# rensonnetg/microstructure_fingerprinting

Hardware: AMD Instinct MI355X
Metric: voxels/sec, 2-fascicle exhaustive NNLS, 782-atom x 200-measurement dictionary (higher is better)
Workload: dtype f64 (pairs ranked on split-f16 MFMA, short list re-evaluated in f64); 1 GPU; C2: 100000 voxels/GPU, 2 fascicles, 782 atoms x 200 measurements; voxels_per_gpu=100000, global_voxels=100000, atoms=782, measurements=200, ranks_in_group=1

## Files before the change

microstructure_fingerprinting_amd/csrc/fit_k2s.hip:

```cpp
#pragma once
#include "fit_k2.hip"

typedef _Float16 h8 __attribute__((ext_vector_type(8)));
typedef _Float16 h4 __attribute__((ext_vector_type(4)));
typedef float f32x16 __attribute__((ext_vector_type(16)));
typedef float f32x2 __attribute__((ext_vector_type(2)));
typedef float f32x4 __attribute__((ext_vector_type(4)));
typedef int i32x4 __attribute__((ext_vector_type(4)));

#ifndef MFX_S_DC
#define MFX_S_DC 1.5e-5
#endif
template <int KS>
__host__ __device__ constexpr double mfx_s_dc() { return KS <= 13 ? (double)MFX_S_DC : 1.05 * (2.38e-6 + 3.0 * KS * 3.046e-7); }
#define MFX_S_DENMIN 1e-3
#define MFX_S_BOUND 0x40000000
#define MFX_S_GUARD 0.25

__device__ __forceinline__ unsigned long long mfx_nonneg_bits(double x) {
  return (unsigned long long)__double_as_longlong(x > 0.0 ? x : 0.0);
}

template <int CTRL>
__device__ __forceinline__ float mfx_dpp_max_f32(float v) {
// ... 12 lines not shown
  return (double)fmaxf(fmaxf(r0, r1), fmaxf(r2, r3));
}
__device__ __forceinline__ double mfx_rcp_nr(double x) {
  const double r0 = (double)__builtin_amdgcn_rcpf((float)x);
  return fma(r0, fma(-x, r0, 1.0), r0);
}

__device__ __forceinline__ double mfx_readlane_f64(double v, int l) {
  const long long b = __double_as_longlong(v);
  const unsigned lo = (unsigned)__builtin_amdgcn_readlane((int)(b & 0xffffffffll), l);
  const unsigned hi = (unsigned)__builtin_amdgcn_readlane((int)(b >> 32), l);
  return __longlong_as_double((long long)(((unsigned long long)hi << 32) | lo));
}

__device__ __forceinline__ void mfx_split16(float f, _Float16& hi, _Float16& lo) {
  asm("" : "+v"(f));
  const float h = __uint_as_float(__float_as_uint(f) & 0xffffe000u);
  hi = (_Float16)h;
  lo = (_Float16)(f - h);
}

#include "k2s_shared.h"

template <int KS, bool BR = false, int NB = 3, bool XC = false>
__global__ __launch_bounds__(512, 2) void mfx_fit_k2s_kernel(FitK2Args a) {
  constexpr int WG = 512, NW = 8;
  constexpr int MP = KS * 16;
  extern __shared__ double smem[];
  int tid = threadIdx.x;
  const int lane = tid & 63, wave = tid >> 6;
  const int lr = lane & 31, lh = lane >> 5;
  [[maybe_unused]] const int M = a.P.M;
  const int N = a.T.N, ldn = a.T.ldn;
  const int NP = (N + 31) & ~31;
  const int ntiles = NP >> 5;
  const int vox = a.vox_list ? a.vox_list[a.vox_base + blockIdx.x] : a.vox_base + (int)blockIdx.x;

  const K2sLds<KS, NB, BR, XC, NW * 64> L(smem, NP);
  K2S_UNPACK(L);
  const K2sVoxel VX = k2s_prologue<KS, NB, BR, XC, NW * 64, WG>(a, L, vox, tid);
  const double y_sq = VX.y_sq, yx = VX.yx, ramp = VX.ramp, dc_eff = VX.dc_eff, mrg = VX.mrg, etol = VX.etol;
  (void)y_sq; (void)yx;
  const float2* __restrict__ tab32 = a.P.tab32s;
  auto tab32_at = [&](int ro, int n) -> float2 { return *(const float2*)((const char*)tab32 + ((unsigned)(ro + n) << 3)); };
  auto tab32x2_at = [&](int ro, int n) -> f32x4 { return *(const f32x4*)((const char*)tab32 + ((unsigned)(ro + n) << 3)); };
  auto push = [&](double S, int i, int j) { k2s_push(L, a.scap, S, i, j); };

  MFX_STAMP(2);
#ifdef MFX_STAMPS_RND
  if (a.stamps && tid == 0) a.stamps[(size_t)blockIdx.x * 16] = __builtin_amdgcn_s_memtime();
#endif
  double bs1 = 0.0;
  int bn1 = 0;
  const int nrounds = (ntiles + NW - 1) / NW;
#ifdef MFX_EXP_NOAUDIT
  const int aud_key = -1;
#else
  const int aud_key = a.audit ? k2s_audit_key(k2s_audit_hash(vox), (ntiles % NW == 1 && ntiles > 1) ? ntiles - 1 : ntiles, ntiles) : -1;
#endif
  for (int round = 0; round < nrounds; ++round) {
    const bool tail = (ntiles - round * NW == 1) && (ntiles > 1);
    const int rt = tail ? round * NW : round * NW + wave;
    const bool rt_valid = rt < ntiles;
    const int rtc = rt_valid ? rt : 0;
    h8 afh[KS], afl[KS];
    {
      const int n = rtc * 32 + lr;
      const int nn = min(n, ldn - 1);
      double a2 = 0.0, ay = 0.0;
      float um1 = 0.0f;
      if constexpr (XC) um1 = (rt_valid && n < N) ? -s_uf[n] : 0.0f;
      mfx_static_for<0, KS>([&](auto kc) {
        constexpr int ks = decltype(kc)::value;
        float2 d[8];
#pragma unroll
        for (int j = 0; j < 8; ++j) d[j] = tab32_at(s_rs[16 * ks + 8 * lh + j], nn);
        h8 vh, vl;
#pragma unroll
        for (int j = 0; j < 8; ++j) {
          float fv = fmaf(d[j].y, s_t0f[16 * ks + 8 * lh + j], d[j].x);
          fv = rt_valid ? fv : 0.0f;
          if constexpr (XC) {
            if constexpr (ks == KS - 1) { if (j == 7) fv = lh ? um1 : fv; }
          } else {
            const double fd = (double)fv;
            a2 = fma(fd, fd, a2);
            ay = fma((double)s_yf[16 * ks + 8 * lh + j], fd, ay);
          }
          _Float16 x, y;
// ... 36 lines not shown
#ifdef MFX_STAMPS_RND
    int dbg_flagged = 0, dbg_groups = 0;
#endif
    const float DCF = XC ? (float)((mfx_s_dc<KS>() + 2e-6) * ramp) * (1.0f + 2e-7f)
                         : (float)mfx_s_dc<KS>() + 2e-6f;
    auto pq_of = [&](float z, float rth, float& P, float& Q) {
      P = fminf(1.0f, fmaxf(z, 0.0f) * rth);
      Q = __builtin_amdgcn_sqrtf(fmaxf(0.0f, fmaf(-P, P, 1.0f) - 1.2e-7f)) * (1.0f - 3e-7f);
    };
    unsigned long long sc_thr = 0ull;
    float sc_z2 = 0.0f, sc_s = 0.0f;
    auto scan_pre = [&](int ct) {
      const int j = ct * 32 + lr;
      sc_thr = s_thr[0];
      sc_z2 = s_Zf[NP + j];
      sc_s = s_cs[NP + j];
    };
#ifdef MFX_STAMPS_SCAN
    int dbg_calls = 0;
#define MFX_SCAN_T(k) do { if (a.stamps && round == 0 && dbg_calls == 1 && wave == 0 && lane == 0) a.stamps[(size_t)blockIdx.x * 16 + (k)] = __builtin_amdgcn_s_memtime(); } while (0)
#else
#define MFX_SCAN_T(k) do { } while (0)
#endif
    auto scan_main = [&](const f32x16& acc, int ct) {
#ifdef MFX_STAMPS_SCAN
      ++dbg_calls;
#endif
      MFX_SCAN_T(0);
      {
        if (((rt << 8) | ct) == aud_key) {
          const unsigned h = k2s_audit_hash(vox);
          const int ga = (h >> 16) & 15;
          float v = acc[0];
#pragma unroll
          for (int g = 1; g < 16; ++g) v = (ga == g) ? acc[g] : v;
          if (lane == (int)((h >> 20) & 63)) ((float*)(s_red + 30))[0] = v;
        }
      }
      const int j = ct * 32 + lr;
      thr = fmax(thr, __longlong_as_double((long long)sc_thr));
      const float rth = __builtin_amdgcn_rsqf(fmaxf((float)thr * (1.0f - 2e-7f), 1e-30f)) * (1.0f + 4e-7f);
      float* pqw = s_pq + wave * 64;
      if (thr > thr_rows) {
        thr_rows = thr;
        if (lane < 32) {
          const float z1 = s_Zf[rtc * 32 + lane], n1 = s_cs[rtc * 32 + lane];
          float P, Q;
          pq_of(z1, rth, P, Q);
          const bool ok = n1 > 0.0f;
          pqw[lane] = ok ? (P + DCF) * n1 : 0.0f;
          pqw[32 + lane] = ok ? Q * ((1.0f - DCF) * n1) : 1e18f;
        }
      }
      const float z2f = sc_z2, n2 = sc_s;
      float P2, Q2;
      pq_of(z2f, rth, P2, Q2);
      const bool colok = n2 > 0.0f;
      const float p2 = colok ? (P2 + DCF) * n2 : -1e18f, q2 = colok ? Q2 * ((1.0f - DCF) * n2) : 1e18f;
      float mm[4];
#pragma unroll
      for (int q = 0; q < 4; ++q) {
        const f32x4 p1q = *(const f32x4*)(pqw + 8 * q + 4 * lh);
        const f32x4 q1q = *(const f32x4*)(pqw + 32 + 8 * q + 4 * lh);
        float t[4];
#pragma unroll
        for (int u = 0; u < 4; ++u) t[u] = fmaf(-q1q[u], q2, fmaf(p1q[u], p2, -acc[4 * q + u]));
        mm[q] = fmaxf(fmaxf(t[0], t[1]), fmaxf(t[2], t[3]));
      }
      MFX_SCAN_T(1);
      if (__any(fmaxf(fmaxf(mm[0], mm[1]), fmaxf(mm[2], mm[3])) >= 0.0f)) {
        MFX_SCAN_T(2);
#ifdef MFX_STAMPS_RND
        ++dbg_flagged;
#endif
        const double z2 = (double)s_Zf[NP + j], n2d = (double)s_cs[NP + j];
#pragma unroll 1
        for (int q = 0; q < 4; ++q) {
          if (!__any(mm[q] >= 0.0f)) continue;
          const f32x4 p1q = *(const f32x4*)(pqw + 8 * q + 4 * lh);
          const f32x4 q1q = *(const f32x4*)(pqw + 32 + 8 * q + 4 * lh);
#pragma unroll 1
          for (int gg = 0; gg < 4; ++gg) {
            const int g = 4 * q + gg;
            if (!__any(fmaf(-q1q[gg], q2, fmaf(p1q[gg], p2, -acc[g])) >= 0.0f)) continue;
#ifdef MFX_STAMPS_RND
            ++dbg_groups;
#endif
            const int i = rt * 32 + (g & 3) + 8 * (g >> 2) + 4 * lh;
            const double n12 = (double)s_cs[i] * n2d;
            const double c = n12 > 0.0 ? (double)acc[g] * mfx_rcp_nr(n12) : 0.0;
            const double z1 = (double)s_Zf[i];
            const double e1 = fma(-c, z2, z1);
            const double e2 = fma(-c, z1, z2);
            const double den = fma(-c, c, 1.0);
            const double num = fma(z2, e2, z1 * e1);
            const bool pos = (e1 > -etol) & (e2 > -etol);
            const bool wellc = (den >= MFX_S_DENMIN) & (c >= 0.0);
            const bool hit = pos & wellc & (fma(-thr, den, num) >= 0.0);
            const bool near = pos & !wellc;
            if (!__any(hit | near)) continue;
            double S = -1.0;
            if (hit) {
              S = num * mfx_rcp_nr(den);
            } else if (near) {
              const double dlo = den - 2.0 * dc_eff - dc_eff * dc_eff;
              const double u1 = fabs(e1) + etol, u2 = fabs(e2) + etol;
              S = (dlo > 0.0 && c > -0.5) ? fmin(fma(z2, z2, u1 * u1 / dlo), fma(z1, z1, u2 * u2 / dlo)) + mrg : 1e300;
            }
            bool feas = hit;
            double q1x = 0.0, q2x = 0.0;
            if constexpr (XC) {
// ... 24 lines not shown
            const double smax = mfx_wave_max_down(fmax(sraise, 0.0));
            if (smax - 2.0 * mrg > thr) {
              thr = smax - 2.0 * mrg;
              if (lane == 0) atomicMax(&s_thr[0], mfx_nonneg_bits(thr));
            }
            if ((hit | near) && slist >= thr) push(slist, i, hit ? j : (j | MFX_S_BOUND));
#ifdef MFX_STAMPS_SCAN
            if (a.stamps && round == 0 && dbg_calls == 1 && wave == 0 && lane == 0) {
              unsigned long long* st = a.stamps + (size_t)blockIdx.x * 16;
              if (st[15] < 8) st[4 + st[15]] = __builtin_amdgcn_s_memtime();
              ++st[15];
            }
#endif
          }
        }
        MFX_SCAN_T(3);
      }
    };
    auto scan_tile = [&](const f32x16& acc, int ct) { scan_pre(ct); scan_main(acc, ct); };

#ifdef MFX_EXP_NOTAIL
    if (tail) continue;
#endif
    if (tail) {
#ifdef MFX_STAMPS_RND
      if (a.stamps && tid == 0 && round < 4) a.stamps[(size_t)blockIdx.x * 16 + 2 * round + 1] = __builtin_amdgcn_s_memtime();
#endif
      thr = __longlong_as_double((long long)s_thr[0]);
      for (int ct = wave; ct < ntiles; ct += NW) {
        const int n = ct * 32 + lr;
        const int nn = min(n, ldn - 1);
        float tail_u2 = 0.0f;
        if constexpr (XC) tail_u2 = s_uf[NP + n];
        f32x16 acc;
#pragma unroll
        for (int g = 0; g < 16; ++g) acc[g] = 0.0f;
        float2 d[2][8];
#pragma unroll
        for (int j = 0; j < 8; ++j) d[0][j] = tab32_at(s_rs[MP + 8 * lh + j], nn);
        mfx_static_for<0, KS>([&](auto kc) {
          constexpr int ks = decltype(kc)::value;
          if constexpr (ks + 1 < KS) {
#pragma unroll
            for (int j = 0; j < 8; ++j) d[(ks + 1) & 1][j] = tab32_at(s_rs[MP + 16 * (ks + 1) + 8 * lh + j], nn);
          }
          h8 bh, bl;
#pragma unroll
          for (int j = 0; j < 8; ++j) {
            _Float16 x, y;
            float fv = fmaf(d[ks & 1][j].y, s_t0f[MP + 16 * ks + 8 * lh + j], d[ks & 1][j].x);
            if constexpr (XC && ks == KS - 1) { if (j == 7) fv = lh ? tail_u2 : fv; }
            mfx_split16(fv, x, y);
            bh[j] = x; bl[j] = y;
          }
          acc = __builtin_amdgcn_mfma_f32_32x32x16_f16(afh[ks], bh, acc, 0, 0, 0);
          acc = __builtin_amdgcn_mfma_f32_32x32x16_f16(afh[ks], bl, acc, 0, 0, 0);
          acc = __builtin_amdgcn_mfma_f32_32x32x16_f16(afl[ks], bh, acc, 0, 0, 0);
          __builtin_amdgcn_sched_barrier(0);
        });
        scan_tile(acc, ct);
      }
      __syncthreads();
#ifdef MFX_STAMPS_RND
      if (a.stamps && tid == 0 && round < 4) a.stamps[(size_t)blockIdx.x * 16 + 2 * round + 2] = __builtin_amdgcn_s_memtime();
#endif
      continue;
    }

    const int grp = wave >> 2, tg = tid & 255;
    static_assert(KS <= 16, "one generation item per thread");
    f32x4 gd[8];
    const int gq = KS * grp + (tg >> 4);
    const bool gact = (tg >> 4) < KS;
    auto gen_load = [&](int ch) {
      const int nn = min(ch * 32 + 2 * (tg & 15), ldn - 2);
      const int q = gact ? gq : KS * grp;
#pragma unroll
      for (int e = 0; e < 8; ++e) gd[e] = tab32x2_at(s_rs[MP + 8 * q + e], nn);
    };
#ifndef MFX_XC_GT
#define MFX_XC_GT 0
#endif
    constexpr bool GT = KS <= 13 && (!XC || MFX_XC_GT);
    float g_t[GT ? 8 : 1];
    if constexpr (GT) {
#pragma unroll
      for (int e = 0; e < 8; ++e) g_t[e] = s_t0f[MP + 8 * (gact ? gq : KS * grp) + e];
    }
    auto gen_store = [&](int ch, int buf) {
      if (gact) {
        const int c0 = 2 * (tg & 15);
        h8 hi0, lo0, hi1, lo1;
// ... 21 lines not shown
#pragma unroll
    for (int g = 0; g < 16; ++g) acc[g] = 0.0f;
    auto mfma_chunk = [&](int buf) {
#pragma unroll
      for (int g = 0; g < 16; ++g) acc[g] = 0.0f;
      const _Float16* bhp = sBh + buf * KS * 512 + lane * 8;
      const _Float16* blp = sBl + buf * KS * 512 + lane * 8;
      h8 bh = *(const h8*)bhp, bl = *(const h8*)blp;
      mfx_static_for<0, KS>([&](auto kc) {
        constexpr int ks = decltype(kc)::value;
        h8 bhn = bh, bln = bl;
        if constexpr (ks + 1 < KS) {
          bhn = *(const h8*)(bhp + (ks + 1) * 512);
          bln = *(const h8*)(blp + (ks + 1) * 512);
        }
        acc = __builtin_amdgcn_mfma_f32_32x32x16_f16(afh[ks], bh, acc, 0, 0, 0);
        acc = __builtin_amdgcn_mfma_f32_32x32x16_f16(afh[ks], bl, acc, 0, 0, 0);
        acc = __builtin_amdgcn_mfma_f32_32x32x16_f16(afl[ks], bh, acc, 0, 0, 0);
        bh = bhn; bl = bln;
        __builtin_amdgcn_sched_barrier(0);
      });
    };

    if (round == 0) MFX_STAMP(3);
#ifdef MFX_STAMPS_RND
    if (a.stamps && tid == 0 && round < 4) a.stamps[(size_t)blockIdx.x * 16 + 2 * round + 1] = __builtin_amdgcn_s_memtime();
#endif
    if constexpr (NB == 3) {
      gen_load(0);
      gen_store(0, 0);
      if (grp == 0) {
        if (ntiles > 1) { gen_load(1); gen_store(1, 1); }
        if (ntiles > 2) gen_load(2);
      } else if (ntiles > 1) {
        gen_load(1);
      }
      __syncthreads();
      if (round == 0) MFX_STAMP(4);
      thr = __longlong_as_double((long long)s_thr[0]);
      int b0 = 0;
#ifdef MFX_EXP_NOGEN
      const bool exp_gen = round == 0;
#else
      constexpr bool exp_gen = true;
#endif
      for (int c = 0; c <= ntiles; ++c) {
#ifdef MFX_STAMPS_HS
#ifndef MFX_HS_ROUND
#define MFX_HS_ROUND 1
#define MFX_HS_C0 10
#endif
        if (a.stamps && round == MFX_HS_ROUND && c >= MFX_HS_C0 && c < MFX_HS_C0 + 16 && tid == 0) a.stamps[(size_t)blockIdx.x * 16 + c - MFX_HS_C0] = __builtin_amdgcn_s_memtime();
#endif
        const int b1 = b0 == 2 ? 0 : b0 + 1, b2 = b1 == 2 ? 0 : b1 + 1;
        if (grp == 0) {
          if (c < ntiles) {
            if (rt_valid) { mfma_chunk(b0); scan_pre(c); }
            if (exp_gen && c + 2 < ntiles) gen_store(c + 2, b2);
            if (rt_valid) scan_main(acc, c);
            if (exp_gen && c + 3 < ntiles) gen_load(c + 3);
          }
        } else {
          if (c >= 1 && rt_valid) scan_pre(c - 1);
          if (exp_gen && c + 1 < ntiles) gen_store(c + 1, b1);
          if (c >= 1 && rt_valid) scan_main(acc, c - 1);
          if (exp_gen && c + 2 < ntiles) gen_load(c + 2);
          if (c < ntiles && rt_valid) mfma_chunk(b0);
        }
        asm volatile("s_waitcnt lgkmcnt(0)\n\ts_barrier" ::: "memory");
        b0 = b1;
      }
    } else {
      gen_load(0);
      gen_store(0, 0);
      if (grp == 1 && ntiles > 1) { gen_load(1); gen_store(1, 1); }
      __syncthreads();
      if (round == 0) MFX_STAMP(4);
      thr = __longlong_as_double((long long)s_thr[0]);
      for (int hs = 0; hs <= 2 * ntiles; ++hs) {
        if ((hs & 1) == grp) {
          const int c = (hs - grp) >> 1;
          if (c < ntiles) {
            if (c + 1 + grp < ntiles) gen_load(c + 1 + grp);
            if (rt_valid) mfma_chunk(c & 1);
          }
        } else {
          const int c = (hs - 1 - grp) >> 1;
          if (c >= 0 && c < ntiles) {
            if (c + 1 + grp < ntiles) gen_store(c + 1 + grp, (c + 1 + grp) & 1);
            if (rt_valid) scan_tile(acc, c);
          }
        }
        __syncthreads();
      }
    }
    if (round == 0) MFX_STAMP(5);
#ifdef MFX_STAMPS_RND
    if (a.stamps && tid == 0 && round < 4) a.stamps[(size_t)blockIdx.x * 16 + 2 * round + 2] = __builtin_amdgcn_s_memtime();
    if (a.stamps && lane == 0 && round < 3) atomicAdd(&a.stamps[(size_t)blockIdx.x * 16 + 9 + round], (unsigned long long)dbg_flagged + ((unsigned long long)dbg_groups << 32));
#endif
  }
  k2s_finish<KS, NB, BR, XC, NW * 64, WG>(a, L, VX, vox, wave, lane, bs1, bn1);
}
```

microstructure_fingerprinting_amd/csrc/k2s_launch.h:

```cpp
#pragma once
#include "mfx_host.h"
#include "fit_k2s.hip"

template <int KS, bool BR, int NB>
static int launch_k2s_t(const FitK2Args& a, int nvox, hipStream_t st) {
  MfxThread& T = mfx_thread();
  const size_t lds = mfx_k2s_lds_bytes(KS, a.T.N, BR, NB);
  auto kern = mfx_fit_k2s_kernel<KS, BR, NB>;
  HIPCHK(hipFuncSetAttribute((const void*)kern, hipFuncAttributeMaxDynamicSharedMemorySize, (int)lds));
  StreamMem fbm(st);
  HIPCHK(fbm.alloc(sizeof(int) * ((size_t)nvox + 8)));
  int* fb = fbm.as<int>();
  HIPCHK(hipMemsetAsync(fb, 0, 8 * sizeof(int), st));
  if (int rc = mfx_prof_begin(st)) return rc;
  FitK2Args aa = a;
  aa.stamps = T.stamps;
  aa.fb_count = fb;
  aa.fb_list = fb + 8;
  aa.audit = fb + 2;
  aa.scap = T.k2s_cap ? T.k2s_cap : MFX_S_CAP;
  hipLaunchKernelGGL(kern, dim3(nvox), dim3(512), lds, st, aa);
  HIPCHK(hipGetLastError());
  if (int rc = mfx_prof_end(st)) return rc;
  FitK2Args ab = a;
  ab.vox_list = fb + 8;
  ab.list_count = fb;
  if (int rc = mfx_launch_k2_f64(ab, nvox, st, false)) return rc;
  if (int rc = mfx_fb_accumulate(fb, 2, st)) return rc;
  return mfx_fb_accumulate_audit(fb + 2, st);
}

#define MFX_K2S_TU(KS_, NAME_)                                                            \
  int NAME_(const FitK2Args& a, int nvox, hipStream_t st, bool br, int NB) {              \
    if (NB == 3) return br ? launch_k2s_t<KS_, true, 3>(a, nvox, st) : launch_k2s_t<KS_, false, 3>(a, nvox, st); \
    return br ? launch_k2s_t<KS_, true, 2>(a, nvox, st) : launch_k2s_t<KS_, false, 2>(a, nvox, st);              \
  }
```

microstructure_fingerprinting_amd/csrc/k2s_shared.h:

```cpp
#pragma once

template <int KS, int NB, bool BR, bool XC, int PQF>
struct K2sLds {
  static constexpr int MP = KS * 16;
  double* smem;
  _Float16* sBh;
  _Float16* sBl;
  double* s_y;
  double* s_t0;
  double* s_red;
  Cand* s_cand;
  unsigned long long* s_thr;
  int* s_r0;
  int* s_cnt;
  float* s_t0f;
  float* s_Zf;
  float* s_cs;
  float* s_yf;
  float* s_pq;
  double* s_t1;
  double* s_tG;
  double* s_dG;
  int* s_r1;
  int* s_rs;
  int* s_evl4;
  float* s_xf;
  float* s_uf;
  __device__ __forceinline__ K2sLds(double* smem_, int NP) : smem(smem_) {
    sBh = (_Float16*)smem;
    sBl = sBh + NB * KS * 512;
    s_y = (double*)(sBl + NB * KS * 512);
    s_t0 = s_y + MP;
    s_red = s_t0 + 2 * MP;
    s_cand = (Cand*)(s_red + 32);
    s_thr = (unsigned long long*)(s_cand + MFX_S_CAP);
    s_r0 = (int*)(s_thr + 2);
    s_cnt = s_r0 + 2 * MP;
    s_t0f = (float*)(s_cnt + 4);
    s_Zf = s_t0f + 2 * MP;
    s_cs = s_Zf + 2 * NP;
    s_yf = s_cs + 2 * NP;
    s_pq = s_yf + MP;
    s_t1 = (double*)(s_pq + PQF);
    s_tG = s_t1 + (BR ? 2 * MP : 0);
    s_dG = s_tG + (BR ? MP : 0);
    s_r1 = (int*)(s_dG + (BR ? MP : 0));
    s_rs = BR ? s_r1 + 2 * MP : s_r0;
    s_evl4 = s_r1 + (BR ? 4 * MP : 0);
    s_xf = (float*)(s_evl4 + (KS < 8 ? MFX_S_CAP : 0));
    s_uf = s_xf + (XC ? MP : 0);
  }
};
#define K2S_UNPACK(L) \
  [[maybe_unused]] _Float16* const sBh = (L).sBh; \
  [[maybe_unused]] _Float16* const sBl = (L).sBl; \
  [[maybe_unused]] double* const s_y = (L).s_y; \
  [[maybe_unused]] double* const s_t0 = (L).s_t0; \
  [[maybe_unused]] double* const s_red = (L).s_red; \
  [[maybe_unused]] Cand* const s_cand = (L).s_cand; \
  [[maybe_unused]] unsigned long long* const s_thr = (L).s_thr; \
  [[maybe_unused]] int* const s_r0 = (L).s_r0; \
  [[maybe_unused]] int* const s_cnt = (L).s_cnt; \
  [[maybe_unused]] float* const s_t0f = (L).s_t0f; \
  [[maybe_unused]] float* const s_Zf = (L).s_Zf; \
  [[maybe_unused]] float* const s_cs = (L).s_cs; \
  [[maybe_unused]] float* const s_yf = (L).s_yf; \
  [[maybe_unused]] float* const s_pq = (L).s_pq; \
  [[maybe_unused]] double* const s_t1 = (L).s_t1; \
  [[maybe_unused]] double* const s_tG = (L).s_tG; \
  [[maybe_unused]] double* const s_dG = (L).s_dG; \
  [[maybe_unused]] int* const s_r1 = (L).s_r1; \
  [[maybe_unused]] int* const s_rs = (L).s_rs; \
  [[maybe_unused]] int* const s_evl4 = (L).s_evl4; \
// ... 11 lines not shown

__device__ __forceinline__ unsigned k2s_audit_hash(int vox) {
  unsigned h = (unsigned)vox * 2654435761u;
  h ^= h >> 15; h *= 2246822519u; h ^= h >> 13; h *= 3266489917u; h ^= h >> 16;
  return h;
}
__device__ __forceinline__ int k2s_audit_key(unsigned h, int ntiles_reg, int ntiles) {
  return ntiles_reg > 0 ? (int)(((h & 0xffu) % (unsigned)ntiles_reg) << 8) | (int)(((h >> 8) & 0xffu) % (unsigned)ntiles) : -1;
}

template <class LDS>
__device__ __forceinline__ void k2s_push(const LDS& L, int scap, double S, int i, int j) {
  const int slot = atomicAdd(&L.s_cnt[0], 1);
  const int idx = slot & (scap - 1);
  if (slot >= scap) {
    const double old = L.s_cand[idx].score;
    atomicMax(&L.s_thr[1], mfx_nonneg_bits(fmin(old, 1e300)));
  }
  L.s_cand[idx].score = S;
  L.s_cand[idx].i = i;
  L.s_cand[idx].j = j;
}

template <int KS, int NB, bool BR, bool XC, int PQF, int WG>
__device__ __forceinline__ K2sVoxel k2s_prologue(const FitK2Args& a, const K2sLds<KS, NB, BR, XC, PQF>& L, const int vox, const int tid) {
  constexpr int MP = KS * 16, NW = WG / 64;
  const int lane = tid & 63, wave = tid >> 6;
  const int M = a.P.M, N = a.T.N, ldn = a.T.ldn;
  const int NP = (N + 31) & ~31;
  [[maybe_unused]] double* const smem = L.smem;
  K2S_UNPACK(L);

  MFX_STAMP(0);
  const double* __restrict__ yv = a.Y + (size_t)vox * M;
  const double* __restrict__ pk = a.peaks + (size_t)vox * a.peaks_ld;
  for (int m = tid; m < MP; m += WG) { const double v = (m < M) ? yv[m] : 0.0; s_y[m] = v; s_yf[m] = (float)v; }
  for (int idx = tid; idx < 2 * MP; idx += WG) {
    const int k = idx / MP, m = idx - k * MP;
    RowDesc rd;
    rd.r0 = a.T.P; rd.t0 = 0.0; rd.r1 = -1; rd.t1 = 0.0;
    if (m < M) rd = mfx_row_desc(a.T, a.P, m, pk[3 * k], pk[3 * k + 1], pk[3 * k + 2]);
    s_r0[idx] = rd.r0 * ldn;
    s_t0[idx] = rd.t0;
    if constexpr (!BR) {
      s_t0f[idx] = (float)rd.t0;
    } else {
      s_r1[idx] = rd.r1 < 0 ? -1 : rd.r1 * ldn;
      s_t1[idx] = rd.t1;
// ... 190 lines not shown
          if (s2 > s || (s2 == s && n2 < n)) { s = s2; n = n2; }
        }
        best1 = fmax(best1, s);
        if (!XC && s > 0.0) {
          const int slot = s_cnt[0]++;
          s_cand[slot].score = s + mrg;
          s_cand[slot].i = k ? 0 : n;
          s_cand[slot].j = (k ? n : 0) | MFX_S_BOUND;
        }
      }
      s_thr[0] = mfx_nonneg_bits(best1 - mrg);
#ifdef MFX_STAMPS_RND
      if (a.stamps) {
        const double t0 = __longlong_as_double((long long)a.stamps[(size_t)blockIdx.x * 16 + 15]);
        if (t0 > best1 - mrg) s_thr[0] = mfx_nonneg_bits(t0);
      }
#endif
    }
  }
  __syncthreads();
  return K2sVoxel{y_sq, yx, ramp, dc_eff, mrg, etol};
}

template <int KS, int NB, bool BR, bool XC, int PQF, int WG>
__device__ __forceinline__ void k2s_finish(const FitK2Args& a, const K2sLds<KS, NB, BR, XC, PQF>& L, const K2sVoxel& VX, const int vox,
                                           const int wave, const int lane, const double bs1, const int bn1) {
  constexpr int MP = KS * 16, NW = WG / 64;
  const int M = a.P.M, N = a.T.N;
  const int NP = (N + 31) & ~31;
  const double2* __restrict__ tab = a.T.tab;
  [[maybe_unused]] double* const smem = L.smem;
  K2S_UNPACK(L);
  const double y_sq = VX.y_sq, yx = VX.yx, mrg = VX.mrg;
  auto push = [&](double S, int i, int j) { k2s_push(L, a.scap, S, i, j); };
  auto tab_at = [&](int ro, int n) -> double2 { return *(const double2*)((const char*)tab + ((unsigned)(ro + n) << 4)); };
  auto elem = [&](int k, int m, int n) -> double {
    const double2 e = tab_at(s_r0[k * MP + m], n);
    const double v0 = e.y * s_t0[k * MP + m] + e.x;
    if constexpr (BR) {
      const int r1 = s_r1[k * MP + m];
      if (r1 < 0) return v0;
      const double2 f = tab_at(r1, n);
      const double v1 = f.y * s_t1[k * MP + m] + f.x;
      const double sl = (v1 - v0) / s_dG[m];
      return sl * s_tG[m] + v0;
    }
    return v0;
  };
// ... 355 lines not shown
```

microstructure_fingerprinting_amd/csrc/mfx_api.hip:

```cpp
#include "mfx_host.h"

#include <algorithm>
#include <chrono>
#include <cmath>
#include <cstdarg>
#include <cstdio>
#include <cstdlib>
#include <cstring>
#include <memory>
#include <string>
#include <vector>

#include "fit_small.hip"
#include "extras.hip"
#include "rotate.hip"
#include "solve_generic.hip"
#include "solve_k3.hip"
#include "fit_k3.hip"
#include "mc_average.hip"
#include "cleanup.hip"
#include "mfx_device.h"

MfxThread& mfx_thread() {
  static thread_local MfxThread t;
// ... 452 lines not shown
  }
  return plan_upload(t, M, g, slo, shi, tG, dG, 1, out);
}

extern "C" void mfx_plan_destroy(mfx_plan* p) {
  if (!p) return;
  (void)hipSetDevice(p->t->device);
  delete p;
}

extern "C" int mfx_plan_status(const mfx_plan* p, void* stream) {
  if (!p) return fail(MFX_ERR_ARG, "mfx_plan_status: null plan");
  if (int rc = require_device(p->t->device)) return rc;
  int st[4] = {0, 0, 0, 0};
  HIPCHK(hipMemcpyAsync(st, p->dstatus, sizeof(st), hipMemcpyDeviceToHost, (hipStream_t)stream));
  HIPCHK(hipStreamSynchronize((hipStream_t)stream));
  if (st[0] == 0) return MFX_OK;
  HIPCHK(hipMemsetAsync(p->dstatus, 0, sizeof(st), (hipStream_t)stream));
  if (st[0] & MFX_ST_DIR_NORM)
    return fail(MFX_ERR_DIR_NORM, "Orientation vector of the new signal must have unit norm (voxel %d of the batch).", st[1]);
  return fail(MFX_ERR_HIP, "fit kernels reported status 0x%x", st[0]);
}

size_t mfx_k2s_lds_bytes(int KS, int N, bool bracket, int NB) {
  const size_t MP = (size_t)KS * 16, NP = ((size_t)N + 31) / 32 * 32;
  return (size_t)2 * NB * KS * 512 * 2 + 8 * (MP + 2 * MP + 32) + sizeof(Cand) * MFX_S_CAP + 16 + 4 * (2 * MP + 4) + 4 * (2 * MP) + 4 * (4 * NP) + 4 * MP + 4 * 8 * 64 +
         (bracket ? 48 * MP : 0) + (KS < 8 ? 4 * MFX_S_CAP : 0);
}

size_t mfx_k2sx_lds_bytes(int KS, int N, bool bracket, int NB) {
  const size_t MP = (size_t)KS * 16, NP = ((size_t)N + 31) / 32 * 32;
  return mfx_k2s_lds_bytes(KS, N, bracket, NB) + 4 * MP + 8 * NP;
}

size_t mfx_k2w_lds_bytes(int KS, int N, bool bracket, int NB, int TL) {
  const size_t MP = (size_t)KS * 16, NP = ((size_t)N + 31) / 32 * 32;
  return (size_t)2 * NB * KS * 512 * 2 + 8 * (MP + 2 * MP + 32) + sizeof(Cand) * MFX_S_CAP + 16 + 4 * (2 * MP + 4) + 4 * (2 * MP) + 4 * (4 * NP) + 4 * MP +
         4 * 4 * TL * 64 + (bracket ? 48 * MP : 0) + (KS < 8 ? 4 * MFX_S_CAP : 0);
}

size_t mfx_k2wx_lds_bytes(int KS, int N, bool bracket, int NB, int TL) {
  const size_t MP = (size_t)KS * 16, NP = ((size_t)N + 31) / 32 * 32;
  return mfx_k2w_lds_bytes(KS, N, bracket, NB, TL) + 4 * MP + 8 * NP;
}

static int launch_k2(const FitK2Args& a, int nvox, hipStream_t st) {
  MfxThread& T = mfx_thread();
  if (T.k2_screen < 0) { const char* e = getenv("MFX_K2_SCREEN"); T.k2_screen = (e && e[0] == '0') ? 0 : 1; }
  if (T.k2_wide < 0) { const char* e = getenv("MFX_K2_WIDE"); T.k2_wide = e ? (e[0] == '1' ? 1 : (e[0] == '0' ? 0 : 2)) : 2; }
  const int M = a.P.M;
// ... 1091 lines not shown
```

microstructure_fingerprinting_amd/csrc/mfx_host.h:

```cpp
#pragma once
#include "../../include/mfx.h"

#include <hip/hip_runtime.h>

#include <string>
#include <vector>

#include "fit_k2.hip"
#include "fit_k2x.hip"

#define MFX_NCOUNTERS 12

struct MfxThread {
  std::string err;
  hipEvent_t ev0 = nullptr, ev1 = nullptr;
  int ev_launches = 0;
  bool ev_valid = false;
  bool profiling = false;
  unsigned long long* stamps = nullptr;
  int k2_pipe = -1;
  int k2_maxc = MFX_MAXC;
  int k2x_maxc = MFX_XMAXC;
  int k2s_nb = 0;
  int k2s_cap = 0;
// ... 59 lines not shown
  explicit StreamMem(hipStream_t s_) : s(s_) {}
  StreamMem(const StreamMem&) = delete;
  StreamMem& operator=(const StreamMem&) = delete;
  ~StreamMem() { if (p) mfx_scratch_free(p, s); }
  hipError_t alloc(size_t bytes) { return mfx_scratch_alloc(&p, bytes, s); }
  template <class T> T* as() const { return (T*)p; }
};

int mfx_prof_begin(hipStream_t st);
int mfx_prof_end(hipStream_t st);
int mfx_fb_begin(hipStream_t st);
int mfx_fb_accumulate(const int* d_counters, int n, hipStream_t st, int offset = 0);
int mfx_fb_accumulate_audit(const int* d_audit, hipStream_t st);
int mfx_fb_end(hipStream_t st);

void mfx_plan_view(const mfx_plan* p, TablesDev* T, PlanDev* P, int* device);

int mfx_solve_dense_scratch_bytes(int M, int K, int N, int has_csf, size_t* bytes);
int mfx_solve_dense_dev(const double* d_A, int M, int K, int N, int has_csf, const double* d_y, int maxfasc, int csf_on,
                        double* d_row, const int* run_if, void* d_scratch, hipStream_t st);

int mfx_launch_k2_f64(const FitK2Args& a, int nvox, hipStream_t st, bool record_events);
bool mfx_k2_f64_fits(const FitK2Args& a);
size_t mfx_k2s_lds_bytes(int KS, int N, bool bracket, int NB);
int mfx_launch_k2s_ks4(const FitK2Args& a, int nvox, hipStream_t st, bool br, int NB);
int mfx_launch_k2s_ks8(const FitK2Args& a, int nvox, hipStream_t st, bool br, int NB);
int mfx_launch_k2s_ks13(const FitK2Args& a, int nvox, hipStream_t st, bool br, int NB);
int mfx_launch_k2s_ks16(const FitK2Args& a, int nvox, hipStream_t st, bool br, int NB);
size_t mfx_k2sx_lds_bytes(int KS, int N, bool bracket, int NB);
int mfx_launch_k2sx_ks8(const FitK2Args& a, int nvox, hipStream_t st, bool br);
int mfx_launch_k2sx_ks13(const FitK2Args& a, int nvox, hipStream_t st, bool br);
size_t mfx_k2w_lds_bytes(int KS, int N, bool bracket, int NB, int TL);
size_t mfx_k2wx_lds_bytes(int KS, int N, bool bracket, int NB, int TL);
int mfx_launch_k2wx_ks24(const FitK2Args& a, int nvox, hipStream_t st, bool br);
int mfx_launch_k2wx_ks35(const FitK2Args& a, int nvox, hipStream_t st, bool br);
int mfx_launch_k2w_ks13(const FitK2Args& a, int nvox, hipStream_t st, bool br);
int mfx_launch_k2w_ks16(const FitK2Args& a, int nvox, hipStream_t st, bool br);
int mfx_launch_k2w_ks24(const FitK2Args& a, int nvox, hipStream_t st, bool br);
int mfx_launch_k2w_ks35(const FitK2Args& a, int nvox, hipStream_t st, bool br);
int mfx_launch_k2x(const FitK2XArgs& a, int nvox, hipStream_t st);
```

Baseline: 1.110 million voxels/s.

## Fold the final partial row tile into the last full round via 16x16 MFMA

When the atom count leaves one leftover row tile of at most 16 rows after full 8-wave rounds, the kernel drops the separate tail round. Instead it precomputes that remainder's split-f16 row images, norms and correlations in the prologue, on the last wave. The remainder's pairs are then scored during the last regular round with small 16x16x32 MFMA units, spread across waves, each followed by the usual scan. This is meant to remove the poorly utilised tail round, at the cost of extra LDS, extra per-wave pq buffers and more divergent scan code.

```diff
diff --git a/microstructure_fingerprinting_amd/csrc/fit_k2s.hip b/microstructure_fingerprinting_amd/csrc/fit_k2s.hip
--- a/microstructure_fingerprinting_amd/csrc/fit_k2s.hip
+++ b/microstructure_fingerprinting_amd/csrc/fit_k2s.hip
@@ -58,13 +58,17 @@
 
 #include "k2s_shared.h"
 
-template <int KS, bool BR = false, int NB = 3, bool XC = false>
+template <int KS, bool BR = false, int NB = 3, bool XC = false, bool RF = false>
 __global__ __launch_bounds__(512, 2) void mfx_fit_k2s_kernel(FitK2Args a) {
+  static_assert(!RF || (NB == 3 && !XC && KS <= 13), "remainder fold: three chunk images, no extra column, KS <= 13");
   constexpr int WG = 512, NW = 8;
   constexpr int MP = KS * 16;
+  constexpr int KK = (KS + 1) / 2;
   extern __shared__ double smem[];
   int tid = threadIdx.x;
-  const int lane = tid & 63, wave = tid >> 6;
+  int lane_ = tid & 63, wave_ = tid >> 6;
+  if constexpr (RF) asm("" : "+v"(lane_), "+v"(wave_));
+  const int lane = lane_, wave = wave_;
   const int lr = lane & 31, lh = lane >> 5;
   [[maybe_unused]] const int M = a.P.M;
   const int N = a.T.N, ldn = a.T.ldn;
@@ -72,9 +76,10 @@
   const int ntiles = NP >> 5;
   const int vox = a.vox_list ? a.vox_list[a.vox_base + blockIdx.x] : a.vox_base + (int)blockIdx.x;
 
-  const K2sLds<KS, NB, BR, XC, NW * 64> L(smem, NP);
+  constexpr int PQF = RF ? NW * (64 + K2S_RF_PQ) : NW * 64;
+  const K2sLds<KS, NB, BR, XC, PQF, RF> L(smem, NP);
   K2S_UNPACK(L);
-  const K2sVoxel VX = k2s_prologue<KS, NB, BR, XC, NW * 64, WG>(a, L, vox, tid);
+  const K2sVoxel VX = k2s_prologue<KS, NB, BR, XC, PQF, WG>(a, L, vox, tid);
   const double y_sq = VX.y_sq, yx = VX.yx, ramp = VX.ramp, dc_eff = VX.dc_eff, mrg = VX.mrg, etol = VX.etol;
   (void)y_sq; (void)yx;
   const float2* __restrict__ tab32 = a.P.tab32s;
@@ -88,19 +93,83 @@
 #endif
   double bs1 = 0.0;
   int bn1 = 0;
-  const int nrounds = (ntiles + NW - 1) / NW;
+  const int nrounds = RF ? (ntiles - 1) / NW : (ntiles + NW - 1) / NW;
+  [[maybe_unused]] const int rbase = (ntiles - 1) * 32;
+  [[maybe_unused]] _Float16* const sRh = L.sRh;
+  [[maybe_unused]] _Float16* const sRl = L.sRl;
+  if constexpr (RF) {
+    if (wave == NW - 1) {
+      const int row = lane & 15, kq = lane >> 4;
+      const int n = rbase + row;
+      const int nn = min(n, ldn - 1);
+      const bool act = n < N;
+      double a2 = 0.0, ay = 0.0;
+      mfx_static_for<0, KK>([&](auto kc) {
+        constexpr int kk = decltype(kc)::value;
+        const int m0 = 32 * kk + 8 * kq;
+        const bool mok = m0 < MP;
+        const int ms = mok ? m0 : MP - 8;
+        float2 d[8];
+#pragma unroll
+        for (int j = 0; j < 8; ++j) d[j] = tab32_at(s_rs[ms + j], nn);
+        h8 vh, vl;
+#pragma unroll
+        for (int j = 0; j < 8; ++j) {
+          float fv = fmaf(d[j].y, s_t0f[ms + j], d[j].x);
+          fv = (act && mok) ? fv : 0.0f;
+          const double fd = (double)fv;
+          a2 = fma(fd, fd, a2);
+          ay = fma((double)s_yf[ms + j], fd, ay);
+          _Float16 x, y;
+          mfx_split16(fv, x, y);
+          vh[j] = x; vl[j] = y;
+        }
+        *(h8*)(sRh + (kk * 64 + lane) * 8) = vh;
+        *(h8*)(sRl + (kk * 64 + lane) * 8) = vl;
+      });
+      a2 += __shfl_xor(a2, 16); ay += __shfl_xor(ay, 16);
+      a2 += __shfl_xor(a2, 32); ay += __shfl_xor(ay, 32);
+      const double nrm = sqrt(a2);
+      const double inv = (act && a2 > 0.0) ? 1.0 / nrm : 0.0;
+      const double z = ay * inv;
+      if (kq == 0) {
+        s_Zf[n] = act ? (float)z : -1e30f;
+        s_cs[n] = (act && a2 > 0.0) ? (float)nrm : 0.0f;
+        s_Zf[n + 16] = -1e30f;
+        s_cs[n + 16] = 0.0f;
+      }
+      if (lane < NW) *(double*)(s_pq + NW * 64 + lane * K2S_RF_PQ + 16) = -1.0;
+      double sb = (act && z > 0.0) ? z * z : 0.0;
+      int nb = n;
+#pragma unroll
+      for (int o = 8; o > 0; o >>= 1) {
+        const double s2 = __shfl_xor(sb, o);
+        const int n2 = __shfl_xor(nb, o);
+        const bool take = (s2 > sb) || (s2 == sb && n2 < nb);
+        sb = take ? s2 : sb;
+        nb = take ? n2 : nb;
+      }
+      sb = mfx_readlane_f64(sb, 0);
+      nb = __builtin_amdgcn_readfirstlane(nb);
+      if (sb > bs1 || (sb == bs1 && sb > 0.0 && nb < bn1)) { bs1 = sb; bn1 = nb; }
+      if (lane == 0 && sb - mrg > 0.0) atomicMax(&s_thr[0], mfx_nonneg_bits(sb - mrg));
+    }
+  }
 #ifdef MFX_EXP_NOAUDIT
   const int aud_key = -1;
 #else
   const int aud_key = a.audit ? k2s_audit_key(k2s_audit_hash(vox), (ntiles % NW == 1 && ntiles > 1) ? ntiles - 1 : ntiles, ntiles) : -1;
 #endif
   for (int round = 0; round < nrounds; ++round) {
-    const bool tail = (ntiles - round * NW == 1) && (ntiles > 1);
+    const bool tail = !RF && (ntiles - round * NW == 1) && (ntiles > 1);
     const int rt = tail ? round * NW : round * NW + wave;
-    const bool rt_valid = rt < ntiles;
+    const bool rt_valid = RF || rt < ntiles;
     const int rtc = rt_valid ? rt : 0;
     h8 afh[KS], afl[KS];
     {
+      int lane_a = lane;
+      if constexpr (RF) asm volatile("" : "+v"(lane_a));
+      const int lr = lane_a & 31, lh = lane_a >> 5;
       const int n = rtc * 32 + lr;
       const int nn = min(n, ldn - 1);
       double a2 = 0.0, ay = 0.0;
@@ -183,12 +252,15 @@
 #else
 #define MFX_SCAN_T(k) do { } while (0)
 #endif
-    auto scan_main = [&](const f32x16& acc, int ct) {
+    auto scan_main = [&](const f32x16& acc, int ct, int remh = -1) {
+      const bool rem = RF && remh >= 0;
+      int ln = lane;
+      if constexpr (RF) asm volatile("" : "+v"(ln));
 #ifdef MFX_STAMPS_SCAN
       ++dbg_calls;
 #endif
       MFX_SCAN_T(0);
-      {
+      if (!rem) {
         if (((rt << 8) | ct) == aud_key) {
           const unsigned h = k2s_audit_hash(vox);
           const int ga = (h >> 16) & 15;
@@ -198,19 +270,22 @@
           if (lane == (int)((h >> 20) & 63)) ((float*)(s_red + 30))[0] = v;
         }
       }
-      const int j = ct * 32 + lr;
+      const int j = rem ? ct * 32 + 16 * remh + (ln & 15) : ct * 32 + lr;
+      if (rem) { sc_thr = s_thr[0]; sc_z2 = s_Zf[NP + j]; sc_s = s_cs[NP + j]; }
       thr = fmax(thr, __longlong_as_double((long long)sc_thr));
       const float rth = __builtin_amdgcn_rsqf(fmaxf((float)thr * (1.0f - 2e-7f), 1e-30f)) * (1.0f + 4e-7f);
-      float* pqw = s_pq + wave * 64;
-      if (thr > thr_rows) {
-        thr_rows = thr;
-        if (lane < 32) {
-          const float z1 = s_Zf[rtc * 32 + lane], n1 = s_cs[rtc * 32 + lane];
+      float* pqw = s_pq + (rem ? NW * 64 + wave * K2S_RF_PQ : wave * 64);
+      const double thr_made = rem ? *(const double*)(pqw + 16) : thr_rows;
+      if (thr > thr_made) {
+        if (rem) { if (ln == 0) *(double*)(pqw + 16) = thr; } else thr_rows = RF ? mfx_readlane_f64(thr, 0) : thr;
+        if (ln < (rem ? 16 : 32)) {
+          const int n1i = (rem ? rbase : rtc * 32) + ln;
+          const float z1 = s_Zf[n1i], n1 = s_cs[n1i];
           float P, Q;
           pq_of(z1, rth, P, Q);
           const bool ok = n1 > 0.0f;
-          pqw[lane] = ok ? (P + DCF) * n1 : 0.0f;
-          pqw[32 + lane] = ok ? Q * ((1.0f - DCF) * n1) : 1e18f;
+          pqw[ln] = ok ? (P + DCF) * n1 : 0.0f;
+          pqw[32 + ln] = ok ? Q * ((1.0f - DCF) * n1) : 1e18f;
         }
       }
       const float z2f = sc_z2, n2 = sc_s;
@@ -218,15 +293,24 @@
       pq_of(z2f, rth, P2, Q2);
       const bool colok = n2 > 0.0f;
       const float p2 = colok ? (P2 + DCF) * n2 : -1e18f, q2 = colok ? Q2 * ((1.0f - DCF) * n2) : 1e18f;
+      auto row_of = [&](int l) { return rem ? 4 * (l >> 4) : 4 * (l >> 5); };
+      const int qs = rem ? 0 : 8;
       float mm[4];
+      auto pq_at = [&](const float* prow, int q) -> const float* {
+        if constexpr (RF) return prow + qs * q;
+        else return pqw + 8 * q + 4 * lh;
+      };
+      {
+      const float* prow = pqw + row_of(ln);
 #pragma unroll
       for (int q = 0; q < 4; ++q) {
-        const f32x4 p1q = *(const f32x4*)(pqw + 8 * q + 4 * lh);
-        const f32x4 q1q = *(const f32x4*)(pqw + 32 + 8 * q + 4 * lh);
+        const f32x4 p1q = *(const f32x4*)pq_at(prow, q);
+        const f32x4 q1q = *(const f32x4*)(pq_at(prow, q) + 32);
         float t[4];
 #pragma unroll
         for (int u = 0; u < 4; ++u) t[u] = fmaf(-q1q[u], q2, fmaf(p1q[u], p2, -acc[4 * q + u]));
         mm[q] = fmaxf(fmaxf(t[0], t[1]), fmaxf(t[2], t[3]));
+      }
       }
       MFX_SCAN_T(1);
       if (__any(fmaxf(fmaxf(mm[0], mm[1]), fmaxf(mm[2], mm[3])) >= 0.0f)) {
@@ -235,11 +319,15 @@
         ++dbg_flagged;
 #endif
         const double z2 = (double)s_Zf[NP + j], n2d = (double)s_cs[NP + j];
+        int l2 = lane;
+        if constexpr (RF) asm volatile("" : "+v"(l2));
+        [[maybe_unused]] const float* prow = pqw + row_of(l2);
+        [[maybe_unused]] const int irow = (rem ? rbase : rt * 32) + row_of(l2);
 #pragma unroll 1
         for (int q = 0; q < 4; ++q) {
           if (!__any(mm[q] >= 0.0f)) continue;
-          const f32x4 p1q = *(const f32x4*)(pqw + 8 * q + 4 * lh);
-          const f32x4 q1q = *(const f32x4*)(pqw + 32 + 8 * q + 4 * lh);
+          const f32x4 p1q = *(const f32x4*)pq_at(prow, q);
+          const f32x4 q1q = *(const f32x4*)(pq_at(prow, q) + 32);
 #pragma unroll 1
           for (int gg = 0; gg < 4; ++gg) {
             const int g = 4 * q + gg;
@@ -247,7 +335,8 @@
 #ifdef MFX_STAMPS_RND
             ++dbg_groups;
 #endif
-            const int i = rt * 32 + (g & 3) + 8 * (g >> 2) + 4 * lh;
+            int i = rt * 32 + (g & 3) + 8 * (g >> 2) + 4 * lh;
+            if constexpr (RF) i = irow + (g & 3) + 8 * (g >> 2);
             const double n12 = (double)s_cs[i] * n2d;
             const double c = n12 > 0.0 ? (double)acc[g] * mfx_rcp_nr(n12) : 0.0;
             const double z1 = (double)s_Zf[i];
@@ -318,7 +407,7 @@
 #ifdef MFX_EXP_NOTAIL
     if (tail) continue;
 #endif
-    if (tail) {
+    if constexpr (!RF) if (tail) {
 #ifdef MFX_STAMPS_RND
       if (a.stamps && tid == 0 && round < 4) a.stamps[(size_t)blockIdx.x * 16 + 2 * round + 1] = __builtin_amdgcn_s_memtime();
 #endif
@@ -363,7 +452,7 @@
       continue;
     }
 
-    const int grp = wave >> 2, tg = tid & 255;
+    const int grp = wave >> 2, tg = RF ? ((wave & 3) << 6) | lane : tid & 255;
     static_assert(KS <= 16, "one generation item per thread");
     f32x4 gd[8];
     const int gq = KS * grp + (tg >> 4);
@@ -431,6 +520,65 @@
       });
     };
 
+    auto rem_unit = [&](int half, int buf) {
+      if constexpr (RF) {
+        int ln = lane;
+        asm volatile("" : "+v"(ln));
+        const int kq = ln >> 4, col = 16 * half + (ln & 15);
+        const _Float16* bhp = sBh + buf * KS * 512;
+        const _Float16* blp = sBl + buf * KS * 512;
+        f32x4 r = {0.0f, 0.0f, 0.0f, 0.0f};
+        auto boff = [&](auto kc) {
+          constexpr int kk = decltype(kc)::value;
+          int q = 4 * kk + kq;
+          if constexpr (4 * kk + 3 > 2 * KS - 1) q = min(q, 2 * KS - 1);
+          return (q * 32 + col) * 8;
+        };
+        const int o0 = boff(std::integral_constant<int, 0>{});
+        h8 bh = *(const h8*)(bhp + o0), bl = *(const h8*)(blp + o0);
+        const _Float16* rhp = sRh + ln * 8;
+        const _Float16* rlp = sRl + ln * 8;
+        h8 ah = *(const h8*)rhp, al = *(const h8*)rlp;
+        mfx_static_for<0, KK>([&](auto kc) {
+          constexpr int kk = decltype(kc)::value;
+          h8 bhn = bh, bln = bl, ahn = ah, aln = al;
+          if constexpr (kk + 1 < KK) {
+            const int o1 = boff(std::integral_constant<int, kk + 1>{});
+            bhn = *(const h8*)(bhp + o1); bln = *(const h8*)(blp + o1);
+            ahn = *(const h8*)(rhp + (kk + 1) * 512); aln = *(const h8*)(rlp + (kk + 1) * 512);
+          }
+          r = __builtin_amdgcn_mfma_f32_16x16x32_f16(ah, bh, r, 0, 0, 0);
+          r = __builtin_amdgcn_mfma_f32_16x16x32_f16(ah, bl, r, 0, 0, 0);
+          r = __builtin_amdgcn_mfma_f32_16x16x32_f16(al, bh, r, 0, 0, 0);
+          bh = bhn; bl = bln; ah = ahn; al = aln;
+          __builtin_amdgcn_sched_barrier(0);
+        });
+#pragma unroll
+        for (int g = 0; g < 16; ++g) acc[g] = g < 4 ? r[g] : 1e30f;
+      }
+    };
+#ifndef MFX_RF_DEAL
+#define MFX_RF_DEAL 0
+#endif
+    auto rem_half = [&](int c) -> int {
+      if constexpr (RF) {
+        if (MFX_RF_DEAL == 1 && nrounds > 1) return (round >= nrounds - 2 && wave == (c & 7)) ? round - (nrounds - 2) : -1;
+        return (round == nrounds - 1 && (wave >> 1) == (c & 3)) ? (wave & 1) : -1;
+      }
+      return -1;
+    };
+    auto scan_both = [&](int ct, int c, int buf) {
+      if constexpr (RF) {
+        const int half = c < ntiles ? rem_half(c) : -1;
+        const int p0 = ct >= 0 ? 0 : 1, p1 = half >= 0 ? 2 : 1;
+#pragma unroll 1
+        for (int p = p0; p < p1; ++p) {
+          if (p == 1) rem_unit(half, buf);
+          scan_main(acc, p == 1 ? c : ct, p == 1 ? half : -1);
+        }
+      }
+    };
+
     if (round == 0) MFX_STAMP(3);
 #ifdef MFX_STAMPS_RND
     if (a.stamps && tid == 0 && round < 4) a.stamps[(size_t)blockIdx.x * 16 + 2 * round + 1] = __builtin_amdgcn_s_memtime();
@@ -466,13 +614,15 @@
           if (c < ntiles) {
             if (rt_valid) { mfma_chunk(b0); scan_pre(c); }
             if (exp_gen && c + 2 < ntiles) gen_store(c + 2, b2);
-            if (rt_valid) scan_main(acc, c);
+            if constexpr (RF) scan_both(c, c, b0);
+            else if (rt_valid) scan_main(acc, c);
             if (exp_gen && c + 3 < ntiles) gen_load(c + 3);
           }
         } else {
           if (c >= 1 && rt_valid) scan_pre(c - 1);
           if (exp_gen && c + 1 < ntiles) gen_store(c + 1, b1);
-          if (c >= 1 && rt_valid) scan_main(acc, c - 1);
+          if constexpr (RF) scan_both(c >= 1 ? c - 1 : -1, c, b0);
+          else if (c >= 1 && rt_valid) scan_main(acc, c - 1);
           if (exp_gen && c + 2 < ntiles) gen_load(c + 2);
           if (c < ntiles && rt_valid) mfma_chunk(b0);
         }
@@ -509,5 +659,7 @@
     if (a.stamps && lane == 0 && round < 3) atomicAdd(&a.stamps[(size_t)blockIdx.x * 16 + 9 + round], (unsigned long long)dbg_flagged + ((unsigned long long)dbg_groups << 32));
 #endif
   }
-  k2s_finish<KS, NB, BR, XC, NW * 64, WG>(a, L, VX, vox, wave, lane, bs1, bn1);
+  int wave_fin = wave;
+  if constexpr (RF) asm volatile("" : "+v"(wave_fin));
+  k2s_finish<KS, NB, BR, XC, PQF, WG>(a, L, VX, vox, wave_fin, lane, bs1, bn1);
 }
diff --git a/microstructure_fingerprinting_amd/csrc/k2s_launch.h b/microstructure_fingerprinting_amd/csrc/k2s_launch.h
--- a/microstructure_fingerprinting_amd/csrc/k2s_launch.h
+++ b/microstructure_fingerprinting_amd/csrc/k2s_launch.h
@@ -2,11 +2,11 @@
 #include "mfx_host.h"
 #include "fit_k2s.hip"
 
-template <int KS, bool BR, int NB>
+template <int KS, bool BR, int NB, bool RF = false>
 static int launch_k2s_t(const FitK2Args& a, int nvox, hipStream_t st) {
   MfxThread& T = mfx_thread();
-  const size_t lds = mfx_k2s_lds_bytes(KS, a.T.N, BR, NB);
-  auto kern = mfx_fit_k2s_kernel<KS, BR, NB>;
+  const size_t lds = mfx_k2s_lds_bytes(KS, a.T.N, BR, NB, RF);
+  auto kern = mfx_fit_k2s_kernel<KS, BR, NB, false, RF>;
   HIPCHK(hipFuncSetAttribute((const void*)kern, hipFuncAttributeMaxDynamicSharedMemorySize, (int)lds));
   StreamMem fbm(st);
   HIPCHK(fbm.alloc(sizeof(int) * ((size_t)nvox + 8)));
@@ -30,8 +30,19 @@
   return mfx_fb_accumulate_audit(fb + 2, st);
 }
 
+template <int KS>
+static bool k2s_fold_applies(const FitK2Args& a, bool br, int NB) {
+  const int N = a.T.N, ntiles = (N + 31) / 32;
+  return NB == 3 && KS <= 13 && ntiles > 1 && ntiles % 8 == 1 && N - 32 * (ntiles - 1) <= 16 &&
+         mfx_k2s_lds_bytes(KS, N, br, 3, true) <= 160 * 1024;
+}
+
 #define MFX_K2S_TU(KS_, NAME_)                                                            \
   int NAME_(const FitK2Args& a, int nvox, hipStream_t st, bool br, int NB) {              \
+    if constexpr (KS_ <= 13) {                                                            \
+      if (k2s_fold_applies<KS_>(a, br, NB))                                               \
+        return br ? launch_k2s_t<KS_, true, 3, true>(a, nvox, st) : launch_k2s_t<KS_, false, 3, true>(a, nvox, st); \
+    }                                                                                     \
     if (NB == 3) return br ? launch_k2s_t<KS_, true, 3>(a, nvox, st) : launch_k2s_t<KS_, false, 3>(a, nvox, st); \
     return br ? launch_k2s_t<KS_, true, 2>(a, nvox, st) : launch_k2s_t<KS_, false, 2>(a, nvox, st);              \
   }
diff --git a/microstructure_fingerprinting_amd/csrc/k2s_shared.h b/microstructure_fingerprinting_amd/csrc/k2s_shared.h
--- a/microstructure_fingerprinting_amd/csrc/k2s_shared.h
+++ b/microstructure_fingerprinting_amd/csrc/k2s_shared.h
@@ -1,6 +1,7 @@
 #pragma once
 
-template <int KS, int NB, bool BR, bool XC, int PQF>
+#define K2S_RF_PQ 64
+template <int KS, int NB, bool BR, bool XC, int PQF, bool RF = false>
 struct K2sLds {
   static constexpr int MP = KS * 16;
   double* smem;
@@ -26,6 +27,8 @@
   int* s_evl4;
   float* s_xf;
   float* s_uf;
+  _Float16* sRh;
+  _Float16* sRl;
   __device__ __forceinline__ K2sLds(double* smem_, int NP) : smem(smem_) {
     sBh = (_Float16*)smem;
     sBl = sBh + NB * KS * 512;
@@ -49,6 +52,8 @@
     s_evl4 = s_r1 + (BR ? 4 * MP : 0);
     s_xf = (float*)(s_evl4 + (KS < 8 ? MFX_S_CAP : 0));
     s_uf = s_xf + (XC ? MP : 0);
+    sRh = (_Float16*)(s_uf + (XC ? 2 * NP : 0));
+    sRl = sRh + (RF ? (KS + 1) / 2 * 512 : 0);
   }
 };
 #define K2S_UNPACK(L) \
@@ -106,8 +111,8 @@
   L.s_cand[idx].j = j;
 }
 
-template <int KS, int NB, bool BR, bool XC, int PQF, int WG>
-__device__ __forceinline__ K2sVoxel k2s_prologue(const FitK2Args& a, const K2sLds<KS, NB, BR, XC, PQF>& L, const int vox, const int tid) {
+template <int KS, int NB, bool BR, bool XC, int PQF, int WG, bool RF = false>
+__device__ __forceinline__ K2sVoxel k2s_prologue(const FitK2Args& a, const K2sLds<KS, NB, BR, XC, PQF, RF>& L, const int vox, const int tid) {
   constexpr int MP = KS * 16, NW = WG / 64;
   const int lane = tid & 63, wave = tid >> 6;
   const int M = a.P.M, N = a.T.N, ldn = a.T.ldn;
@@ -344,8 +349,8 @@
   return K2sVoxel{y_sq, yx, ramp, dc_eff, mrg, etol};
 }
 
-template <int KS, int NB, bool BR, bool XC, int PQF, int WG>
-__device__ __forceinline__ void k2s_finish(const FitK2Args& a, const K2sLds<KS, NB, BR, XC, PQF>& L, const K2sVoxel& VX, const int vox,
+template <int KS, int NB, bool BR, bool XC, int PQF, int WG, bool RF = false>
+__device__ __forceinline__ void k2s_finish(const FitK2Args& a, const K2sLds<KS, NB, BR, XC, PQF, RF>& L, const K2sVoxel& VX, const int vox,
                                            const int wave, const int lane, const double bs1, const int bn1) {
   constexpr int MP = KS * 16, NW = WG / 64;
   const int M = a.P.M, N = a.T.N;
diff --git a/microstructure_fingerprinting_amd/csrc/mfx_api.hip b/microstructure_fingerprinting_amd/csrc/mfx_api.hip
--- a/microstructure_fingerprinting_amd/csrc/mfx_api.hip
+++ b/microstructure_fingerprinting_amd/csrc/mfx_api.hip
@@ -498,10 +498,10 @@
   return fail(MFX_ERR_HIP, "fit kernels reported status 0x%x", st[0]);
 }
 
-size_t mfx_k2s_lds_bytes(int KS, int N, bool bracket, int NB) {
+size_t mfx_k2s_lds_bytes(int KS, int N, bool bracket, int NB, bool fold) {
   const size_t MP = (size_t)KS * 16, NP = ((size_t)N + 31) / 32 * 32;
   return (size_t)2 * NB * KS * 512 * 2 + 8 * (MP + 2 * MP + 32) + sizeof(Cand) * MFX_S_CAP + 16 + 4 * (2 * MP + 4) + 4 * (2 * MP) + 4 * (4 * NP) + 4 * MP + 4 * 8 * 64 +
-         (bracket ? 48 * MP : 0) + (KS < 8 ? 4 * MFX_S_CAP : 0);
+         (bracket ? 48 * MP : 0) + (KS < 8 ? 4 * MFX_S_CAP : 0) + (fold ? (size_t)2 * ((KS + 1) / 2) * 512 * 2 + 4 * 8 * 64 : 0);
 }
 
 size_t mfx_k2sx_lds_bytes(int KS, int N, bool bracket, int NB) {
diff --git a/microstructure_fingerprinting_amd/csrc/mfx_host.h b/microstructure_fingerprinting_amd/csrc/mfx_host.h
--- a/microstructure_fingerprinting_amd/csrc/mfx_host.h
+++ b/microstructure_fingerprinting_amd/csrc/mfx_host.h
@@ -105,7 +105,7 @@
 
 int mfx_launch_k2_f64(const FitK2Args& a, int nvox, hipStream_t st, bool record_events);
 bool mfx_k2_f64_fits(const FitK2Args& a);
-size_t mfx_k2s_lds_bytes(int KS, int N, bool bracket, int NB);
+size_t mfx_k2s_lds_bytes(int KS, int N, bool bracket, int NB, bool fold = false);
 int mfx_launch_k2s_ks4(const FitK2Args& a, int nvox, hipStream_t st, bool br, int NB);
 int mfx_launch_k2s_ks8(const FitK2Args& a, int nvox, hipStream_t st, bool br, int NB);
 int mfx_launch_k2s_ks13(const FitK2Args& a, int nvox, hipStream_t st, bool br, int NB);
```

Result: no change. 1.102 million voxels/s (-0.7%).
